# mailgun/gubernator

Measured on AMD Instinct MI355X. Metric: rate-limit decisions/sec (kernel path, inputs resident in HBM), higher is better.
Workload: dtype int64

## Files before the change

gubernator_amd/csrc/guber_front.h:

```cpp
#pragma once
#include "guber_kernels_wire.h"

constexpr uint32_t FRONT_ONE_PAIR_MAX = 49152;
struct guber_front {
    std::mutex mu;
    int device = 0;
    std::vector<guber_engine*> eng;
    std::vector<hipStream_t> streams;
    std::vector<int> stream_of;
    const guber::WireEnc* enc_hook = nullptr;
    hipStream_t rs = nullptr, rs2 = nullptr, os = nullptr, last_os = nullptr; int n_own_streams = 1; bool out_on_eval = false; uint32_t out_delay = 0, one_pair_max = FRONT_ONE_PAIR_MAX; bool rs_borrowed = false;
    uint32_t cap = 0, depth = 0, max_key = 0;
    uint32_t seq = 0;
    DevBuf<uint16_t> rt_table, rt_exs; DevBuf<uint64_t> rt_exh; RouteRule rule{}; bool have_rule = false;
    struct Slot {
        DevBuf<uint8_t> mem; CohBuf<FrontHost> host;
        FrIn in{};
        uint8_t *o_status = nullptr, *o_err = nullptr; int64_t *o_limit = nullptr, *o_remaining = nullptr, *o_reset = nullptr;
        hipEvent_t ev_in = nullptr, ev_out = nullptr, ev_a = nullptr; bool out_recorded = false;
        std::vector<std::unique_ptr<EvalHook>> hooks;
        CohBuf<uint8_t> h_margs; DevBuf<uint8_t> d_margs;
        uint32_t seq = 0, n = 0;
        int64_t gen = -1;
        bool dispatched = false;
    };
    std::vector<Slot> slots;
    uint64_t generations = 0, forced_flushes = 0, host_waits = 0; double host_wait_ms = 0;
    bool pre_routed = false;
    struct GenSpan { hipEvent_t a, b; };
    std::vector<GenSpan> gen_spans;
};

static size_t front_col(size_t bytes) { return (bytes + 63) & ~(size_t)63; }
struct FrontGen { guber_batch_t b; uint32_t key_stride = 0; const uint32_t* key_len = nullptr; };

extern "C" void guber_front_destroy(guber_front_t* f) {
    if (!f) return;
    (void)hipSetDevice(f->device);
    for (hipStream_t st : {f->rs, f->rs2, f->os}) if (st) (void)hipStreamSynchronize(st);
    for (auto st : f->streams) (void)hipStreamSynchronize(st);
    for (auto& s : f->slots) {
        s.mem.release(); s.host.release(); s.h_margs.release(); s.d_margs.release();
        if (s.ev_in) (void)hipEventDestroy(s.ev_in);
        if (s.ev_out) (void)hipEventDestroy(s.ev_out);
        for (auto& h : s.hooks) if (h && h->ev) (void)hipEventDestroy(h->ev);
    }
    f->rt_table.release(); f->rt_exs.release(); f->rt_exh.release();
    if (f->rs2 && f->rs2 != f->rs) (void)hipStreamDestroy(f->rs2);
    if (f->os && f->os != f->rs) (void)hipStreamDestroy(f->os);
    if (f->rs && !f->rs_borrowed) (void)hipStreamDestroy(f->rs);
    delete f;
}

static int front_set_rule(guber_front* f, const guber_route_rule_t* rule) {
    if (rule->n_shards == 0 || rule->per == 0 || !rule->table || rule->n_shards > 4096 || (rule->ex_cells & (rule->ex_cells - 1)) ||
        (rule->ex_n && (!rule->ex_hash || !rule->ex_shard || rule->ex_n >= rule->ex_cells)))
        return fail(GUBER_E_INVALID_ARG, "malformed route rule");
    const size_t slots = (size_t)rule->n_shards * rule->per, cells = rule->ex_cells ? rule->ex_cells : 1;
    if (f->rt_table.ensure(slots) || f->rt_exh.ensure(cells) || f->rt_exs.ensure(cells)) return GUBER_E_NOMEM;
    hipError_t he = hipStreamSynchronize(f->rs);
    if (he == hipSuccess && f->rs2) he = hipStreamSynchronize(f->rs2);
    if (he == hipSuccess) he = hipMemcpy(f->rt_table.p, rule->table, slots * 2, hipMemcpyHostToDevice);
    if (he == hipSuccess && rule->ex_n) he = hipMemcpy(f->rt_exh.p, rule->ex_hash, cells * 8, hipMemcpyHostToDevice);
    if (he == hipSuccess && rule->ex_n) he = hipMemcpy(f->rt_exs.p, rule->ex_shard, cells * 2, hipMemcpyHostToDevice);
    if (he != hipSuccess) { f->have_rule = false; return fail(GUBER_E_HIP, "guber_front: rule upload", he); }
    f->rule = RouteRule{rule->n_shards, rule->per, rule->ex_cells, rule->ex_n, rule->global_engine, rule->step, rule->inv_step, rule->inv_sub,
                        f->rt_table.p, (const unsigned long long*)f->rt_exh.p, f->rt_exs.p};
    f->have_rule = true;
    return 0;
}

extern "C" int guber_front_create(guber_engine_t* const* engines, uint32_t n_engines, const guber_route_rule_t* rule, uint32_t max_n,
                                  uint32_t depth, guber_front_t** out) {
    if (!engines || !out || !n_engines || n_engines > (uint32_t)MULTI_MEM_MAX) return fail(GUBER_E_INVALID_ARG, "1 .. 16 engines per front");
    if (n_engines > 1 && !rule) return fail(GUBER_E_INVALID_ARG, "a front over several engines needs the placement's rule");
    if (max_n == 0 || max_n > FR_MAX_N) return fail(GUBER_E_BATCH_TOO_LARGE, "a generation holds at most 4 194 304 requests");
    if (depth == 0) depth = 4;
    if (depth < 3 || depth > 16) return fail(GUBER_E_INVALID_ARG, "3 .. 16 generations in flight");
    std::unique_ptr<guber_front, void (*)(guber_front*)> f(new guber_front(), [](guber_front* p) { guber_front_destroy(p); });
    for (uint32_t j = 0; j < n_engines; ++j) {
        guber_engine* e = engines[j];
        if (!e) return fail(GUBER_E_INVALID_ARG, "null engine");
        if (e->device != engines[0]->device) return fail(GUBER_E_INVALID_ARG, "the engines of a front live on one device");
        for (uint32_t q = 0; q < j; ++q) if (engines[q] == e) return fail(GUBER_E_INVALID_ARG, "an engine twice in one front");
        f->eng.push_back(e);
        int si = -1;
        for (size_t q = 0; q < f->streams.size(); ++q) if (f->streams[q] == e->stream) si = (int)q;
        if (si < 0) { si = (int)f->streams.size(); f->streams.push_back(e->stream); }
        f->stream_of.push_back(si);
        f->max_key = j == 0 ? e->max_key : std::min(f->max_key, e->max_key);
    }
    f->device = engines[0]->device; f->cap = max_n; f->depth = depth;
    if (hipSetDevice(f->device) != hipSuccess) return fail(GUBER_E_HIP, "hipSetDevice");
    HIPCHK(hipStreamCreateWithFlags(&f->rs, hipStreamNonBlocking));
    f->n_own_streams = 1;
    if (const char* v = guber_lab_env("GUBER_FRONT_STREAMS")) f->n_own_streams = std::max(1, std::min(3, atoi(v)));
    f->out_on_eval = true;
    if (const char* v = guber_lab_env("GUBER_FRONT_OUT_ON_EVAL")) f->out_on_eval = atoi(v) != 0;
    if (const char* v = guber_lab_env("GUBER_FRONT_OUT_DELAY")) f->out_delay = (uint32_t)std::max(0, std::min(2, atoi(v)));
    if (const char* v = guber_lab_env("GUBER_FRONT_ONE_PAIR_MAX")) f->one_pair_max = (uint32_t)strtoul(v, nullptr, 10);
    f->rs2 = f->os = f->rs;
    if (f->n_own_streams >= 2) HIPCHK(hipStreamCreateWithFlags(&f->os, hipStreamNonBlocking));
    if (f->n_own_streams >= 3) HIPCHK(hipStreamCreateWithFlags(&f->rs2, hipStreamNonBlocking));
    if (rule) { const int rc = front_set_rule(f.get(), rule); if (rc) return rc; }
    else f->rule = RouteRule{1, 1, 0, 0, -1, 0, 0, 0, nullptr, nullptr, nullptr};
    const size_t cap = max_n, tiles = (cap + FR_TILE - 1) / FR_TILE;
    f->slots.resize(depth);
    for (auto& s : f->slots) {
        const size_t bytes = 3 * front_col(cap * 4 + 4) + 5 * front_col(cap * 8) + front_col(cap * 4) + 2 * front_col(cap) +
                             3 * front_col(cap * 8) + 2 * front_col(cap) +
                             front_col(cap * FR_KEY_COPY_MAX + 64) +
                             front_col(cap * 2) + 2 * front_col(tiles * MULTI_MEM_MAX * 4) + front_col(sizeof(FrontCtl));
        if (s.mem.ensure(bytes) || s.host.ensure(1)) return GUBER_E_NOMEM;
        if (f->streams.size() == 1 && n_engines > 1 && (s.h_margs.ensure(sizeof(MultiArgsMem)) || s.d_margs.ensure(sizeof(MultiArgsMem)))) return GUBER_E_NOMEM;
        uint8_t* p = s.mem.p;
        FrIn& A = s.in;
        A.d_key_off = (uint32_t*)p; p += front_col(cap * 4 + 4); A.d_key_len = (uint32_t*)p; p += front_col(cap * 4 + 4); A.d_fwd = (uint32_t*)p; p += front_col(cap * 4 + 4);
        A.d_hits = (int64_t*)p; p += front_col(cap * 8); A.d_limit = (int64_t*)p; p += front_col(cap * 8); A.d_duration = (int64_t*)p; p += front_col(cap * 8);
        A.d_burst = (int64_t*)p; p += front_col(cap * 8); A.d_created_at = (int64_t*)p; p += front_col(cap * 8);
        A.d_behavior = (uint32_t*)p; p += front_col(cap * 4); A.d_algorithm = p; p += front_col(cap); A.d_is_owner = p; p += front_col(cap);
        s.o_limit = (int64_t*)p; p += front_col(cap * 8); s.o_remaining = (int64_t*)p; p += front_col(cap * 8); s.o_reset = (int64_t*)p; p += front_col(cap * 8);
        s.o_status = p; p += front_col(cap); s.o_err = p; p += front_col(cap);
        A.d_keys = p; p += front_col(cap * FR_KEY_COPY_MAX + 64);
        A.er = (uint16_t*)p; p += front_col(cap * 2);
        A.tile_cnt = (uint32_t*)p; p += front_col(tiles * MULTI_MEM_MAX * 4); A.tile_base = (uint32_t*)p; p += front_col(tiles * MULTI_MEM_MAX * 4);
        A.ctl = (FrontCtl*)p; p += front_col(sizeof(FrontCtl));
        A.host = s.host.p;
        memset((void*)s.host.p, 0, sizeof(FrontHost));
        HIPCHK(hipMemsetAsync(A.ctl, 0, sizeof(FrontCtl), f->rs));
        HIPCHK(hipMemsetAsync(A.d_keys, 0, front_col(cap * FR_KEY_COPY_MAX + 64), f->rs));
        HIPCHK(hipEventCreateWithFlags(&s.ev_in, hipEventDisableTiming));
        HIPCHK(hipEventCreateWithFlags(&s.ev_out, hipEventDisableTiming));
        for (size_t q = 0; q < f->streams.size(); ++q) {
            s.hooks.emplace_back(new EvalHook());
            HIPCHK(hipEventCreateWithFlags(&s.hooks.back()->ev, hipEventDisableTiming));
            s.hooks.back()->st = f->streams[q];
        }
    }
    HIPCHK(hipStreamSynchronize(f->rs));
    *out = f.release();
    return GUBER_OK;
}

static int front_route_on(guber_front* f, hipStream_t st) {
    std::lock_guard<std::mutex> lk(f->mu);
    if (f->generations || f->pre_routed || f->n_own_streams != 1) return fail(GUBER_E_INVALID_ARG, "guber_front: the routing stream is chosen before the first generation");
    if (hipSetDevice(f->device) != hipSuccess) return fail(GUBER_E_HIP, "hipSetDevice");
    HIPCHK(hipStreamSynchronize(f->rs));
    HIPCHK(hipStreamDestroy(f->rs));
    f->rs = f->rs2 = f->os = st; f->rs_borrowed = true;
    return 0;
}

extern "C" int guber_front_set_rule(guber_front_t* f, const guber_route_rule_t* rule) {
    if (!f || !rule) return fail(GUBER_E_INVALID_ARG, "null argument");
    std::lock_guard<std::mutex> lk(f->mu);
    if (hipSetDevice(f->device) != hipSuccess) return fail(GUBER_E_HIP, "hipSetDevice");
    return front_set_rule(f, rule);
}

static int front_route(guber_front* f, guber_front::Slot& s, const FrontGen* fg, int64_t gen) {
    const guber_batch_t* b = &fg->b;
    hipStream_t rs = (gen & 1) ? f->rs2 : f->rs;
    if (s.out_recorded) { HIPCHK(hipStreamWaitEvent(rs, s.ev_out, 0)); s.out_recorded = false; }
    s.gen = gen; s.n = b->n; s.dispatched = false;
    s.seq = ++f->seq ? f->seq : ++f->seq;
    for (auto& h : s.hooks) { h->outstanding.store(1); h->recorded.store(false); }
    if (b->n == 0) return 0;
    FrIn& A = s.in;
    A.n = b->n; A.n_engines = (uint32_t)f->eng.size(); A.max_key = f->max_key; A.seq = s.seq;
    A.key_bytes = b->key_bytes; A.key_off = b->key_off; A.key_stride = fg->key_stride; A.key_len = fg->key_len; A.hits = b->hits; A.limit = b->limit; A.duration = b->duration;
    A.burst = b->burst; A.created_at = b->created_at; A.behavior = b->behavior; A.algorithm = b->algorithm; A.is_owner = b->is_owner;
    A.R = f->rule;
    const uint32_t tiles = (b->n + FR_TILE - 1u) / FR_TILE;
    guber_engine* e0 = f->eng[0];
    std::unique_lock<std::mutex> pl(e0->mu, std::defer_lock);
    if (e0->profiling) pl.lock();
    s.ev_a = nullptr;
    if (e0->profiling) { s.ev_a = e0->get_event(); (void)hipEventRecord(s.ev_a, rs); }
    e0->span_begin(KT_FR_COUNT, b->n, rs);
    hipLaunchKernelGGL(k_fr_count, dim3(tiles), dim3(FR_TILE), 0, rs, A);
    e0->span_end();
    e0->span_begin(KT_FR_SCAN, b->n, rs);
    hipLaunchKernelGGL(k_fr_scan, dim3(MULTI_MEM_MAX / 4), dim3(FR_SCAN_T), 0, rs, A, tiles, (tiles + FR_SCAN_T - 1) / FR_SCAN_T);
    e0->span_end();
    e0->span_begin(KT_FR_SCATTER, b->n, rs);
    hipLaunchKernelGGL(k_fr_scatter, dim3(tiles), dim3(256), 0, rs, A);
    e0->span_end();
    if (hipGetLastError() != hipSuccess) return fail(GUBER_E_HIP, "kernel launch");
    HIPCHK(hipEventRecord(s.ev_in, rs));
    return 0;
}

static int front_out(guber_front* f, guber_front::Slot& s, guber_result_t* r) {
    if (s.n == 0) return 0;
    hipStream_t os = f->out_on_eval ? f->streams[(size_t)s.gen % f->streams.size()] : f->os;
    f->last_os = os;
    for (auto& h : s.hooks) if (h->st != os) HIPCHK(hipStreamWaitEvent(os, h->ev, 0));
    FrOut O{};
    O.n = s.n; O.fwd = s.in.d_fwd;
    O.d_status = s.o_status; O.d_err = s.o_err; O.d_limit = s.o_limit; O.d_remaining = s.o_remaining; O.d_reset_time = s.o_reset;
    O.status = r->status; O.err = r->err; O.limit = r->limit; O.remaining = r->remaining; O.reset_time = r->reset_time;
    guber_engine* e0 = f->eng[0];
    std::unique_lock<std::mutex> pl(e0->mu, std::defer_lock);
    if (e0->profiling) pl.lock();
    e0->span_begin(KT_FR_OUT, s.n, os);
    if (f->enc_hook) {
        guber::WireEnc E = *f->enc_hook;
        E.fwd = O.fwd; E.d_status = O.d_status; E.d_err = O.d_err; E.d_limit = O.d_limit; E.d_remaining = O.d_remaining; E.d_reset = O.d_reset_time;
        hipLaunchKernelGGL(guber::k_wire_enc, dim3(E.nrpc), dim3(guber::WE_T), 0, os, E);
    } else
    hipLaunchKernelGGL(k_fr_out, dim3((s.n + FR_TILE - 1u) / FR_TILE), dim3(256), 0, os, O);
    e0->span_end();
    if (s.ev_a) { hipEvent_t evb = e0->get_event(); (void)hipEventRecord(evb, os); f->gen_spans.push_back({s.ev_a, evb}); s.ev_a = nullptr; }
    if (hipGetLastError() != hipSuccess) return fail(GUBER_E_HIP, "kernel launch");
    if (os != f->rs) { HIPCHK(hipEventRecord(s.ev_out, os)); s.out_recorded = true; }
    return 0;
}

static bool front_evals_launched(const guber_front::Slot& s) {
    for (auto& h : s.hooks) if (!h->recorded.load(std::memory_order_acquire)) return false;
    return true;
}

static int front_eval(guber_front* f, const FrontGen* gens, guber_result_t* results, uint32_t count, uint32_t* done, hipEvent_t after = nullptr);
extern "C" int guber_front_eval_dev(guber_front_t* f, const guber_batch_t* gens, guber_result_t* results, uint32_t count, uint32_t* done) {
    if (done) *done = 0;
    if (!f || (count && (!gens || !results))) return fail(GUBER_E_INVALID_ARG, "null argument");
    std::vector<FrontGen> g(count);
    for (uint32_t k = 0; k < count; ++k) {
        const int rc = check_batch_args(&gens[k], &results[k]);
        if (rc) return rc;
        g[k].b = gens[k];
    }
    return front_eval(f, g.data(), results, count, done);
}
static int front_eval(guber_front* f, const FrontGen* gens, guber_result_t* results, uint32_t count, uint32_t* done, hipEvent_t after) {
    if (done) *done = 0;
    for (uint32_t k = 0; k < count; ++k) {
        if (gens[k].b.n > f->cap) return fail(GUBER_E_BATCH_TOO_LARGE, "generation larger than the front was created for");
        if (gens[k].b.greg_expire || gens[k].b.greg_duration) return fail(GUBER_E_INVALID_ARG, "a front takes its calendar intervals from the device");
        if (gens[k].key_stride & 7u) return fail(GUBER_E_INVALID_ARG, "key rows are a multiple of 8 bytes apart");
        clear_aggregates(results[k]);
    }
    std::lock_guard<std::mutex> lk(f->mu);
    if (hipSetDevice(f->device) != hipSuccess) return fail(GUBER_E_HIP, "hipSetDevice");
    const uint32_t ne = (uint32_t)f->eng.size(), D = f->depth, ahead = D - 2;
    PendSet pendset;
    bool any_ep = false;
    for (auto* e : f->eng) any_ep = any_ep || e->fuse_ep;
    PendSet* const ps = any_ep ? &pendset : nullptr;
    struct Dispatching { bool on; Dispatching(bool o) : on(o) { if (on) ++tl_ep_dispatcher; } ~Dispatching() { if (on) --tl_ep_dispatcher; } } dispatching(any_ep);
    uint32_t next_route = 0, next_out = 0, enq = 0;
    int rc = 0;
    uint64_t fp[4] = {0, 0, 0, 0};
    struct FpSpan { uint64_t* a; uint64_t t0; explicit FpSpan(uint64_t* x) : a(x), t0(dp_now()) {} ~FpSpan() { if (g_dprof) *a += dp_now() - t0; } };
    const uint64_t g0 = f->generations;
    auto slot_of = [&](uint32_t k) -> guber_front::Slot& { return f->slots[(g0 + k) % D]; };
    auto drain_outs = [&](uint32_t upto, bool force) -> int {
        while (next_out < upto) {
            guber_front::Slot& s = slot_of(next_out);
            if (!s.dispatched) break;
            if (s.n && !front_evals_launched(s)) {
                if (!force) break;
                f->forced_flushes++;
                const int r2 = pendset.flush_all();
                if (r2) return r2;
                if (!front_evals_launched(s)) return fail(GUBER_E_HIP, "guber_front: an evaluation was not launched");
            }
            const int r3 = front_out(f, s, &results[next_out]);
            if (r3) return r3;
            ++next_out;
            if (done) *done = next_out;
        }
        return 0;
    };
    std::vector<std::vector<GroupItem>> fifo(ne);
    std::vector<EvalHook*> hook_of(ne, nullptr);
    for (uint32_t k = 0; k < count && !rc; ++k) {
        while (next_route < count && next_route <= k + ahead && !rc) {
            if (next_route >= D) { rc = drain_outs(next_route - D + 1, true); if (rc) break; }
            if (next_route == 0 && f->pre_routed) f->pre_routed = false;
            else { FpSpan sp(&fp[0]); rc = front_route(f, slot_of(next_route), &gens[next_route], (int64_t)f->generations + next_route); }
            ++next_route;
        }
        if (rc) break;
        guber_front::Slot& s = slot_of(k);
        const guber_batch_t* b = &gens[k].b;
        if (s.n) {
            auto reported = [&]() {
                for (int q = 0; q <= MULTI_MEM_MAX; ++q)
                    if ((uint32_t)(__atomic_load_n((volatile unsigned long long*)&s.host.p->w[q], __ATOMIC_ACQUIRE) >> 32) != s.seq) return false;
                return true;
            };
            if (!reported()) {
                FpSpan sp(&fp[1]);
                const auto t0 = std::chrono::steady_clock::now();
                f->host_waits++;
                uint32_t spins = 0;
                while (!reported()) {
                    if (++spins > 2000) {
                        std::this_thread::yield();
                        if ((spins & 0x3ffu) == 0 && hipStreamQuery((s.gen & 1) ? f->rs2 : f->rs) != hipErrorNotReady && !reported()) {
                            rc = fail(GUBER_E_HIP, "guber_front: the routing of a generation did not report"); break;
                        }
                    }
                }
                f->host_wait_ms += std::chrono::duration<double, std::milli>(std::chrono::steady_clock::now() - t0).count();
                if (rc) break;
            }
            uint32_t counts[MULTI_MEM_MAX];
            for (int q = 0; q < MULTI_MEM_MAX; ++q) counts[q] = (uint32_t)s.host.p->w[q];
            const bool packed = !((uint32_t)s.host.p->w[MULTI_MEM_MAX] >> 8 & 1u);
            for (auto st : f->streams) { if (hipStreamWaitEvent(st, s.ev_in, 0) != hipSuccess) { rc = fail(GUBER_E_HIP, "hipStreamWaitEvent"); break; } }
            if (rc) break;
            uint32_t base = 0, total = 0;
            for (uint32_t j = 0; j < ne; ++j) {
                fifo[j].clear();
                hook_of[j] = s.hooks[f->stream_of[j]].get();
                const uint32_t nj = counts[j];
                total += nj;
                guber_engine* e = f->eng[j];
                const uint32_t cap_e = std::max<uint32_t>(1u, std::min<uint32_t>(e->fast_cap ? e->fast_cap : e->max_batch, e->max_batch));
                const uint32_t np = (nj + cap_e - 1) / cap_e;
                uint32_t piece = np > 1 ? ((nj + np - 1) / np + 255u) & ~255u : cap_e;
                if (piece > cap_e) piece = cap_e;
                for (uint32_t pos = 0; pos < nj; pos += piece) {
                    const uint32_t len = std::min(piece, nj - pos), d0 = base + pos;
                    const FrIn& A = s.in;
                    BatchView B{len, 0, packed ? A.d_keys : b->key_bytes, A.d_key_off + d0, A.d_hits + d0, A.d_limit + d0, A.d_duration + d0,
                                b->burst ? A.d_burst + d0 : nullptr, b->created_at ? A.d_created_at + d0 : nullptr,
                                A.d_algorithm + d0, A.d_behavior + d0, b->is_owner ? A.d_is_owner + d0 : nullptr, nullptr, nullptr, b->now_ms,
                                0, packed ? nullptr : A.d_key_len + d0};
                    fifo[j].push_back(GroupItem{B, ResultView{s.o_status + d0, s.o_limit + d0, s.o_remaining + d0, s.o_reset + d0, s.o_err + d0}});
                }
                base += nj;
            }
            if (total != s.n) { rc = fail(GUBER_E_HIP, "guber_front: the shares do not add up to the generation"); break; }
            bool one_pair = f->streams.size() == 1 && ne > 1 && s.h_margs.p && s.n <= f->one_pair_max;
            guber_engine* og[MULTI_MEM_MAX]; GroupItem oi[MULTI_MEM_MAX]; int on = 0;
            for (uint32_t j = 0; j < ne && one_pair; ++j) {
                if (fifo[j].empty()) continue;
                one_pair = fifo[j].size() == 1 && can_fuse(f->eng[j], fifo[j][0].B.n);
                og[on] = f->eng[j]; oi[on] = fifo[j][0]; ++on;
            }
            if (one_pair && on > 1) {
                FpSpan sp(&fp[2]);
                rc = pendset.flush_all();
                int r1 = rc ? rc : launch_group_mem(og, oi, on, &enq, (MultiArgsMem*)s.h_margs.p, (MultiArgsMem*)s.d_margs.p);
                if (r1 == 1) r1 = dispatch_rounds(f->eng.data(), ne, fifo, ps, &enq, hook_of.data());
                rc = r1;
            } else { FpSpan sp(&fp[2]); rc = dispatch_rounds(f->eng.data(), ne, fifo, ps, &enq, hook_of.data()); }
        }
        s.dispatched = true;
        for (auto& h : s.hooks) h->launched();
        if (rc) break;
        { FpSpan sp(&fp[3]); rc = drain_outs(k + 1 > f->out_delay ? k + 1 - f->out_delay : 0, false); }
    }
    {
        for (uint32_t k = 0; k < next_route; ++k) {
            guber_front::Slot& s = slot_of(k);
            if (k >= next_out && !s.dispatched) { s.dispatched = true; s.n = 0; for (auto& h : s.hooks) h->launched(); }
        }
        const int rcf = pendset.flush_all();
        if (!rc) rc = rcf;
        const int rco = drain_outs(next_route, true);
        if (!rc) rc = rco;
    }
    f->generations += next_out;
    if (after && !rc && hipEventRecord(after, f->last_os ? f->last_os : f->rs) != hipSuccess) rc = fail(GUBER_E_HIP, "hipEventRecord");
    if (g_dprof && next_out) {
        fprintf(stderr, "[front] %u generations; per generation: routing enqueue %.2f us, waiting for the shares' sizes %.2f, dispatch %.2f, answers %.2f\n", next_out,
                fp[0] / 1e3 / next_out, fp[1] / 1e3 / next_out, fp[2] / 1e3 / next_out, fp[3] / 1e3 / next_out);
        if (tl_dp[6]) fprintf(stderr, "[front dispatch] %llu batches in %llu groups; per batch: wait-for-progress %.2f us, locks %.2f, preludes+plans %.2f, argument blocks %.2f, launches %.2f\n",
                (unsigned long long)tl_dp[6], (unsigned long long)tl_dp[5], tl_dp[0] / 1e3 / tl_dp[6], tl_dp[1] / 1e3 / tl_dp[6], tl_dp[2] / 1e3 / tl_dp[6],
                tl_dp[3] / 1e3 / tl_dp[6], tl_dp[4] / 1e3 / tl_dp[6]);
        for (auto& v : tl_dp) v = 0;
    }
    return rc;
}

static int front_route_ahead(guber_front* f, const FrontGen* g) {
    if (g->b.n > f->cap) return fail(GUBER_E_BATCH_TOO_LARGE, "generation larger than the front was created for");
    if (g->key_stride & 7u) return fail(GUBER_E_INVALID_ARG, "key rows are a multiple of 8 bytes apart");
    std::lock_guard<std::mutex> lk(f->mu);
    if (f->pre_routed) return fail(GUBER_E_INVALID_ARG, "guber_front: a generation is routed ahead already");
    if (hipSetDevice(f->device) != hipSuccess) return fail(GUBER_E_HIP, "hipSetDevice");
    const int rc = front_route(f, f->slots[f->generations % f->depth], g, (int64_t)f->generations);
    if (!rc) f->pre_routed = true;
    return rc;
}
static bool front_routed_ahead_ready(guber_front* f) {
    std::lock_guard<std::mutex> lk(f->mu);
    if (!f->pre_routed) return true;
    guber_front::Slot& s = f->slots[f->generations % f->depth];
    if (s.n == 0) return true;
    for (int q = 0; q <= MULTI_MEM_MAX; ++q)
        if ((uint32_t)(__atomic_load_n((volatile unsigned long long*)&s.host.p->w[q], __ATOMIC_ACQUIRE) >> 32) != s.seq) return false;
    return true;
}

extern "C" int guber_front_synchronize(guber_front_t* f) {
    if (!f) return fail(GUBER_E_INVALID_ARG, "null front");
    std::lock_guard<std::mutex> lk(f->mu);
    if (hipSetDevice(f->device) != hipSuccess) return fail(GUBER_E_HIP, "hipSetDevice");
    for (auto st : f->streams) HIPCHK(hipStreamSynchronize(st));
    for (hipStream_t st : {f->rs, f->rs2, f->os}) HIPCHK(hipStreamSynchronize(st));
    return GUBER_OK;
}

extern "C" int guber_front_latencies(guber_front_t* f, float* us, uint32_t cap, uint32_t* n_out) {
    if (!f || !n_out) return fail(GUBER_E_INVALID_ARG, "null argument");
    std::lock_guard<std::mutex> lk(f->mu);
    if (hipSetDevice(f->device) != hipSuccess) return fail(GUBER_E_HIP, "hipSetDevice");
    HIPCHK(hipStreamSynchronize(f->os));
    uint32_t n = 0;
    guber_engine* e0 = f->eng[0];
    std::lock_guard<std::mutex> lk2(e0->mu);
    for (auto& g : f->gen_spans) {
        float ms = 0;
        if (hipEventElapsedTime(&ms, g.a, g.b) == hipSuccess && us && n < cap) us[n] = ms * 1e3f;
        ++n;
        e0->event_pool.push_back(g.a); e0->event_pool.push_back(g.b);
    }
    f->gen_spans.clear();
    *n_out = n;
    return GUBER_OK;
}

extern "C" void* guber_front_stream(guber_front_t* f) { return f ? (void*)f->os : nullptr; }

extern "C" int guber_front_stats(guber_front_t* f, guber_front_stats_t* out) {
    if (!f || !out) return fail(GUBER_E_INVALID_ARG, "null argument");
    std::lock_guard<std::mutex> lk(f->mu);
    out->generations = f->generations; out->forced_flushes = f->forced_flushes; out->host_waits = f->host_waits;
    out->host_wait_us = (uint64_t)(f->host_wait_ms * 1e3);
    return GUBER_OK;
}
```

gubernator_amd/csrc/guber_kernels_front.h:

```cpp
#pragma once

namespace guber {

constexpr uint32_t FR_PER = 4;
constexpr uint32_t FR_TILE = 256 * FR_PER;
constexpr uint32_t FR_RANK_BITS = 10;
static_assert((1u << FR_RANK_BITS) >= FR_TILE && (MULTI_MEM_MAX << FR_RANK_BITS) <= 65536, "engine and rank share sixteen bits");
constexpr uint32_t FR_SCAN_T = 1024;
constexpr uint32_t FR_SCAN_PER = 4;
constexpr uint32_t FR_MAX_N = FR_SCAN_T * FR_SCAN_PER * FR_TILE;
constexpr uint32_t FR_KEY_COPY_MAX = 32;

struct FrontCtl {
    uint32_t tot[MULTI_MEM_MAX];
    uint32_t ragged_seq;
    uint32_t pad_[15];
};
struct FrontHost { unsigned long long w[MULTI_MEM_MAX + 1]; unsigned long long pad_[15]; };
static_assert(sizeof(FrontHost) == 256, "four lines of pinned memory per slot");

struct FrIn {
    uint32_t n, n_engines, max_key, seq;
    const uint8_t* key_bytes; const uint32_t* key_off;
    uint32_t key_stride; const uint32_t* key_len;
    const int64_t *hits, *limit, *duration, *burst, *created_at; const uint32_t* behavior; const uint8_t *algorithm, *is_owner;
    uint16_t* er; uint32_t* tile_cnt; uint32_t* tile_base; FrontCtl* ctl; FrontHost* host;
    uint32_t *d_key_off, *d_key_len, *d_fwd; int64_t *d_hits, *d_limit, *d_duration, *d_burst, *d_created_at; uint32_t* d_behavior; uint8_t *d_algorithm, *d_is_owner;
    uint8_t* d_keys;
    RouteRule R;
};
static_assert(sizeof(FrIn) <= 4096, "kernel arguments are limited to 4 KB");
__device__ __forceinline__ uint32_t fr_key_off(const FrIn& A, uint32_t i) { return A.key_stride ? i * A.key_stride : A.key_off[i]; }
__device__ __forceinline__ uint32_t fr_key_len(const FrIn& A, uint32_t i, uint32_t off) { return A.key_stride ? A.key_len[i] : A.key_off[i + 1] - off; }
__device__ __forceinline__ uint32_t fr_len0(const FrIn& A) { return A.key_stride ? A.key_len[0] : A.key_off[1] - A.key_off[0]; }

__global__ __launch_bounds__(FR_TILE) void k_fr_count(FrIn A) {
    __shared__ uint32_t wtot[FR_TILE / 64][MULTI_MEM_MAX];
    const uint32_t tid = threadIdx.x, lane = tid & 63u, wave = tid >> 6, i = blockIdx.x * FR_TILE + tid;
    if (tid < (FR_TILE / 64) * MULTI_MEM_MAX) (&wtot[0][0])[tid] = 0u;
    uint32_t e = 0xffu;
    if (i < A.n) {
        const uint32_t len0 = fr_len0(A);
        const uint32_t o0 = A.key_stride ? 0u : A.key_off[0], oend = A.key_stride ? A.n * A.key_stride : A.key_off[A.n];
        const uint32_t off_g = A.key_stride ? i * A.key_stride : o0 + i * len0;
        uint64_t kw[4] = {0, 0, 0, 0};
        const bool spec = len0 != 0 && len0 < 32 && (A.key_stride ? A.key_stride >= 32u : (uint64_t)off_g + 32 <= (uint64_t)oend + 8);
        if (spec) { const uint8_t* kp = A.key_bytes + off_g; kw[0] = ld_key_word(kp); kw[1] = ld_key_word(kp + 8); kw[2] = ld_key_word(kp + 16); kw[3] = ld_key_word(kp + 24); }
        const uint32_t off = fr_key_off(A, i), len = fr_key_len(A, i, off);
        e = 0;
        if (A.R.global_engine >= 0 && A.behavior && (A.behavior[i] & 2u)) e = (uint32_t)A.R.global_engine;
        else if (len != 0 && len <= A.max_key && A.R.n_shards > 1)
            e = route_engine(A.R, (spec && off == off_g && len == len0) ? xxhash64_words4(kw, len, 0) : xxhash64(A.key_bytes + off, len, 0));
        if (e >= A.n_engines) e = 0;
        if (len != len0 || off != off_g || len0 == 0 || len0 > FR_KEY_COPY_MAX) {
            if (__hip_atomic_load(&A.ctl->ragged_seq, __ATOMIC_RELAXED, __HIP_MEMORY_SCOPE_AGENT) != A.seq) atomicExch(&A.ctl->ragged_seq, A.seq);
        }
    }
    __syncthreads();
    unsigned long long same = __ballot(e <= 15u);
#pragma unroll
    for (uint32_t b = 0; b < 4; ++b) { const unsigned long long m = __ballot((e >> b) & 1u); same &= ((e >> b) & 1u) ? m : ~m; }
    if (e > 15u) same = 0ull;
    uint32_t rank = (uint32_t)__popcll(same & ((1ull << lane) - 1ull));
    if (same && rank == 0) wtot[wave][e] = (uint32_t)__popcll(same);
    __syncthreads();
    if (i < A.n) {
        for (uint32_t w = 0; w < wave; ++w) rank += wtot[w][e];
        A.er[i] = (uint16_t)(e << FR_RANK_BITS | rank);
    }
    if (tid < MULTI_MEM_MAX) {
        uint32_t c = 0;
        for (uint32_t w = 0; w < FR_TILE / 64; ++w) c += wtot[w][tid];
        A.tile_cnt[blockIdx.x * MULTI_MEM_MAX + tid] = c;
    }
}

__global__ __launch_bounds__(FR_SCAN_T) void k_fr_scan(FrIn A, uint32_t nt, uint32_t per) {
    __shared__ uint32_t wsum[FR_SCAN_T / 64][4];
    const uint32_t tid = threadIdx.x, lane = tid & 63u, wave = tid >> 6, q = blockIdx.x;
    const uint32_t t0 = tid * per, t1 = t0 + per < nt ? t0 + per : nt;
    uint32_t m0 = 0, m1 = 0, m2 = 0, m3 = 0;
#pragma unroll 1
    for (uint32_t t = t0; t < t1; ++t) { const uint4 v = ((const uint4*)(A.tile_cnt + (size_t)t * MULTI_MEM_MAX))[q]; m0 += v.x; m1 += v.y; m2 += v.z; m3 += v.w; }
    const uint32_t i0 = (uint32_t)wave_incl_scan_i32((int)m0), i1 = (uint32_t)wave_incl_scan_i32((int)m1);
    const uint32_t i2 = (uint32_t)wave_incl_scan_i32((int)m2), i3 = (uint32_t)wave_incl_scan_i32((int)m3);
    if (lane == 63) { wsum[wave][0] = i0; wsum[wave][1] = i1; wsum[wave][2] = i2; wsum[wave][3] = i3; }
    __syncthreads();
    uint32_t e0 = i0 - m0, e1 = i1 - m1, e2 = i2 - m2, e3 = i3 - m3;
    for (uint32_t w = 0; w < wave; ++w) { e0 += wsum[w][0]; e1 += wsum[w][1]; e2 += wsum[w][2]; e3 += wsum[w][3]; }
#pragma unroll 1
    for (uint32_t t = t0; t < t1; ++t) {
        const uint4 v = ((const uint4*)(A.tile_cnt + (size_t)t * MULTI_MEM_MAX))[q];
        ((uint4*)(A.tile_base + (size_t)t * MULTI_MEM_MAX))[q] = make_uint4(e0, e1, e2, e3);
        e0 += v.x; e1 += v.y; e2 += v.z; e3 += v.w;
    }
    if (tid < 4) {
        uint32_t all = 0;
        for (uint32_t w = 0; w < FR_SCAN_T / 64; ++w) all += wsum[w][tid];
        A.ctl->tot[4 * q + tid] = all;
        __hip_atomic_store(&A.host->w[4 * q + tid], (unsigned long long)A.seq << 32 | all, __ATOMIC_RELAXED, __HIP_MEMORY_SCOPE_SYSTEM);
    }
    if (q == 0 && tid == 0) {
        const uint32_t ragged = __hip_atomic_load(&A.ctl->ragged_seq, __ATOMIC_RELAXED, __HIP_MEMORY_SCOPE_AGENT) == A.seq ? 1u : 0u;
        const uint32_t len0 = fr_len0(A);
        __hip_atomic_store(&A.host->w[MULTI_MEM_MAX], (unsigned long long)A.seq << 32 | ragged << 8 | (len0 < 255u ? len0 : 255u), __ATOMIC_RELAXED, __HIP_MEMORY_SCOPE_SYSTEM);
    }
}

__global__ __launch_bounds__(256) void k_fr_scatter(FrIn A) {
    __shared__ uint32_t sbase[MULTI_MEM_MAX];
    if (threadIdx.x < MULTI_MEM_MAX) {
        uint32_t b = 0;
        for (uint32_t k = 0; k < threadIdx.x; ++k) b += A.ctl->tot[k];
        sbase[threadIdx.x] = b;
    }
    __syncthreads();
    const uint32_t tile = blockIdx.x, i0 = tile * FR_TILE + threadIdx.x;
    const bool packed = A.ctl->ragged_seq != A.seq;
    uint32_t er[FR_PER], o0[FR_PER], o1[FR_PER], beh[FR_PER]; int64_t hits[FR_PER], limit[FR_PER], duration[FR_PER]; uint8_t algo[FR_PER];
#pragma unroll
    for (int k = 0; k < FR_PER; ++k) {
        const uint32_t i = i0 + k * 256u;
        if (i >= A.n) { er[k] = 0xffffffffu; continue; }
        er[k] = A.er[i]; o0[k] = fr_key_off(A, i); o1[k] = o0[k] + fr_key_len(A, i, o0[k]);
        hits[k] = A.hits[i]; limit[k] = A.limit[i]; duration[k] = A.duration[i];
        beh[k] = A.behavior ? A.behavior[i] : 0u; algo[k] = A.algorithm ? A.algorithm[i] : (uint8_t)0;
    }
#pragma unroll
    for (int k = 0; k < FR_PER; ++k) {
        const uint32_t i = i0 + k * 256u;
        if (er[k] == 0xffffffffu) continue;
        const uint32_t e = er[k] >> FR_RANK_BITS, rank = er[k] & ((1u << FR_RANK_BITS) - 1u);
        const uint32_t d = sbase[e] + A.tile_base[tile * MULTI_MEM_MAX + e] + rank;
        A.d_fwd[i] = d < A.n ? d : 0u;
        if (d >= A.n) continue;
        A.d_hits[d] = hits[k]; A.d_limit[d] = limit[k]; A.d_duration[d] = duration[k]; A.d_behavior[d] = beh[k]; A.d_algorithm[d] = algo[k];
        if (A.burst) A.d_burst[d] = A.burst[i];
        if (A.created_at) A.d_created_at[d] = A.created_at[i];
        if (A.is_owner) A.d_is_owner[d] = A.is_owner[i];
        if (packed) {
            const uint32_t len = o1[k] - o0[k];
            const uint8_t* src = A.key_bytes + o0[k]; uint8_t* dst = A.d_keys + (size_t)d * len;
            if (len >= 8) {
                uint32_t b = 0;
                for (; b + 8 <= len; b += 8) { const uint64_t w = ld_key_word(src + b); __builtin_memcpy(dst + b, &w, 8); }
                if (b < len) { const uint64_t w = ld_key_word(src + len - 8); __builtin_memcpy(dst + len - 8, &w, 8); }
            } else {
                const uint64_t w = ld_key_word(src);
                for (uint32_t q = 0; q < len; ++q) dst[q] = (uint8_t)(w >> (8 * q));
            }
            A.d_key_off[d] = d * len;
            if (d == A.n - 1) A.d_key_off[A.n] = A.n * len;
        } else {
            A.d_key_off[d] = o0[k]; A.d_key_len[d] = o1[k] - o0[k];
        }
    }
}

struct FrOut {
    uint32_t n; const uint32_t* fwd;
    const uint8_t *d_status, *d_err; const int64_t *d_limit, *d_remaining, *d_reset_time;
    uint8_t *status, *err; int64_t *limit, *remaining, *reset_time;
};
__global__ __launch_bounds__(256) void k_fr_out(FrOut A) {
    const uint32_t i0 = blockIdx.x * FR_TILE + threadIdx.x;
    uint32_t d[FR_PER]; uint8_t st[FR_PER], er[FR_PER]; int64_t l[FR_PER], r[FR_PER], t[FR_PER];
#pragma unroll
    for (int k = 0; k < FR_PER; ++k) d[k] = i0 + k * 256u < A.n ? A.fwd[i0 + k * 256u] : 0xffffffffu;
#pragma unroll
    for (int k = 0; k < FR_PER; ++k) {
        if (d[k] == 0xffffffffu) continue;
        st[k] = A.d_status[d[k]]; er[k] = A.d_err[d[k]]; l[k] = A.d_limit[d[k]]; r[k] = A.d_remaining[d[k]]; t[k] = A.d_reset_time[d[k]];
    }
#pragma unroll
    for (int k = 0; k < FR_PER; ++k) {
        if (d[k] == 0xffffffffu) continue;
        const uint32_t i = i0 + k * 256u;
        A.limit[i] = l[k]; A.remaining[i] = r[k]; A.reset_time[i] = t[k]; A.status[i] = st[k]; A.err[i] = er[k];
    }
}

}
```

Measured before the change: 4.838 billion.

## Stage front scatter and gather through shared memory for coalesced column writes

The scatter and output kernels now compute per-tile engine bases in shared memory and permute each column through a double-buffered LDS staging array. Global reads and writes then land on contiguous sorted destinations instead of random per-element scatter/gather addresses. The output kernel rebuilds the permutation from the engine/rank codes instead of reading the forward index array. This adds barriers and LDS traffic per column, and relies on each tile's destinations being contiguous per engine. Packed keys are assumed to share one fixed length.

```diff
diff --git a/gubernator_amd/csrc/guber_front.h b/gubernator_amd/csrc/guber_front.h
--- a/gubernator_amd/csrc/guber_front.h
+++ b/gubernator_amd/csrc/guber_front.h
@@ -198,7 +198,7 @@
     f->last_os = os;
     for (auto& h : s.hooks) if (h->st != os) HIPCHK(hipStreamWaitEvent(os, h->ev, 0));
     FrOut O{};
-    O.n = s.n; O.fwd = s.in.d_fwd;
+    O.n = s.n; O.er = s.in.er; O.tile_cnt = s.in.tile_cnt; O.tile_base = s.in.tile_base; O.ctl = s.in.ctl;
     O.d_status = s.o_status; O.d_err = s.o_err; O.d_limit = s.o_limit; O.d_remaining = s.o_remaining; O.d_reset_time = s.o_reset;
     O.status = r->status; O.err = r->err; O.limit = r->limit; O.remaining = r->remaining; O.reset_time = r->reset_time;
     guber_engine* e0 = f->eng[0];
@@ -207,7 +207,7 @@
     e0->span_begin(KT_FR_OUT, s.n, os);
     if (f->enc_hook) {
         guber::WireEnc E = *f->enc_hook;
-        E.fwd = O.fwd; E.d_status = O.d_status; E.d_err = O.d_err; E.d_limit = O.d_limit; E.d_remaining = O.d_remaining; E.d_reset = O.d_reset_time;
+        E.fwd = s.in.d_fwd; E.d_status = O.d_status; E.d_err = O.d_err; E.d_limit = O.d_limit; E.d_remaining = O.d_remaining; E.d_reset = O.d_reset_time;
         hipLaunchKernelGGL(guber::k_wire_enc, dim3(E.nrpc), dim3(guber::WE_T), 0, os, E);
     } else
     hipLaunchKernelGGL(k_fr_out, dim3((s.n + FR_TILE - 1u) / FR_TILE), dim3(256), 0, os, O);
diff --git a/gubernator_amd/csrc/guber_kernels_front.h b/gubernator_amd/csrc/guber_kernels_front.h
--- a/gubernator_amd/csrc/guber_kernels_front.h
+++ b/gubernator_amd/csrc/guber_kernels_front.h
@@ -107,77 +107,168 @@
     }
 }
 
+struct FrTile { uint32_t lbase[MULTI_MEM_MAX + 1], dofs[MULTI_MEM_MAX]; };
+__device__ __forceinline__ void fr_tile_bases(FrTile& T, const FrontCtl* ctl, const uint32_t* tile_cnt, const uint32_t* tile_base, uint32_t tile) {
+    const uint32_t e = threadIdx.x;
+    if (e < MULTI_MEM_MAX) {
+        const uint32_t* cnt = tile_cnt + (size_t)tile * MULTI_MEM_MAX;
+        uint32_t s = 0, l = 0;
+        for (uint32_t k = 0; k < e; ++k) { s += ctl->tot[k]; l += cnt[k]; }
+        T.lbase[e] = l; T.dofs[e] = s + tile_base[(size_t)tile * MULTI_MEM_MAX + e] - l;
+        if (e == MULTI_MEM_MAX - 1) T.lbase[MULTI_MEM_MAX] = l + cnt[e];
+    }
+    __syncthreads();
+}
+__device__ __forceinline__ uint32_t fr_engine_of(const FrTile& T, uint32_t j) {
+    uint32_t e = 0;
+#pragma unroll
+    for (uint32_t q = 1; q < MULTI_MEM_MAX; ++q) e += T.lbase[q] <= j ? 1u : 0u;
+    return e;
+}
+__device__ __forceinline__ void fr_sorted_places(const FrTile& T, uint32_t n, uint32_t (&dd)[FR_PER]) {
+    const uint32_t cnt = T.lbase[MULTI_MEM_MAX] < FR_TILE ? T.lbase[MULTI_MEM_MAX] : FR_TILE;
+#pragma unroll
+    for (int k = 0; k < FR_PER; ++k) {
+        const uint32_t j = threadIdx.x + k * 256u, d = T.dofs[fr_engine_of(T, j)] + j;
+        dd[k] = j < cnt && d < n ? d : 0xffffffffu;
+    }
+}
+
 __global__ __launch_bounds__(256) void k_fr_scatter(FrIn A) {
-    __shared__ uint32_t sbase[MULTI_MEM_MAX];
-    if (threadIdx.x < MULTI_MEM_MAX) {
-        uint32_t b = 0;
-        for (uint32_t k = 0; k < threadIdx.x; ++k) b += A.ctl->tot[k];
-        sbase[threadIdx.x] = b;
-    }
-    __syncthreads();
-    const uint32_t tile = blockIdx.x, i0 = tile * FR_TILE + threadIdx.x;
+    __shared__ FrTile T;
+    __shared__ uint64_t stg[2][FR_TILE];
+    const uint32_t tile = blockIdx.x, tid = threadIdx.x, i0 = tile * FR_TILE + tid;
+    fr_tile_bases(T, A.ctl, A.tile_cnt, A.tile_base, tile);
     const bool packed = A.ctl->ragged_seq != A.seq;
-    uint32_t er[FR_PER], o0[FR_PER], o1[FR_PER], beh[FR_PER]; int64_t hits[FR_PER], limit[FR_PER], duration[FR_PER]; uint8_t algo[FR_PER];
+    const uint32_t len0 = fr_len0(A), ko0 = A.key_stride ? 0u : A.key_off[0], kstep = A.key_stride ? A.key_stride : len0;
+    uint32_t p[FR_PER], o0[FR_PER], klen[FR_PER]; uint64_t hits[FR_PER], limit[FR_PER], duration[FR_PER], misc[FR_PER], kw[FR_PER];
+    auto word_at = [](uint32_t w, uint32_t len) { return 8u * w + 8u <= len || len < 8u ? 8u * w : len - 8u; };
 #pragma unroll
     for (int k = 0; k < FR_PER; ++k) {
         const uint32_t i = i0 + k * 256u;
-        if (i >= A.n) { er[k] = 0xffffffffu; continue; }
-        er[k] = A.er[i]; o0[k] = fr_key_off(A, i); o1[k] = o0[k] + fr_key_len(A, i, o0[k]);
-        hits[k] = A.hits[i]; limit[k] = A.limit[i]; duration[k] = A.duration[i];
-        beh[k] = A.behavior ? A.behavior[i] : 0u; algo[k] = A.algorithm ? A.algorithm[i] : (uint8_t)0;
-    }
-#pragma unroll
-    for (int k = 0; k < FR_PER; ++k) {
-        const uint32_t i = i0 + k * 256u;
-        if (er[k] == 0xffffffffu) continue;
-        const uint32_t e = er[k] >> FR_RANK_BITS, rank = er[k] & ((1u << FR_RANK_BITS) - 1u);
-        const uint32_t d = sbase[e] + A.tile_base[tile * MULTI_MEM_MAX + e] + rank;
+        p[k] = 0xffffffffu; o0[k] = klen[k] = 0; hits[k] = limit[k] = duration[k] = misc[k] = kw[k] = 0;
+        if (i >= A.n) continue;
+        const uint32_t er = A.er[i];
+        if (packed) { o0[k] = ko0 + i * kstep; klen[k] = len0; kw[k] = ld_key_word(A.key_bytes + o0[k]); }
+        else { o0[k] = fr_key_off(A, i); klen[k] = fr_key_len(A, i, o0[k]); }
+        hits[k] = (uint64_t)A.hits[i]; limit[k] = (uint64_t)A.limit[i]; duration[k] = (uint64_t)A.duration[i];
+        misc[k] = (A.behavior ? A.behavior[i] : 0u) | (uint64_t)(A.algorithm ? A.algorithm[i] : (uint8_t)0) << 32 | (uint64_t)(A.is_owner ? A.is_owner[i] : (uint8_t)0) << 40;
+        const uint32_t e = er >> FR_RANK_BITS;
+        p[k] = T.lbase[e] + (er & ((1u << FR_RANK_BITS) - 1u));
+        const uint32_t d = T.dofs[e] + p[k];
         A.d_fwd[i] = d < A.n ? d : 0u;
-        if (d >= A.n) continue;
-        A.d_hits[d] = hits[k]; A.d_limit[d] = limit[k]; A.d_duration[d] = duration[k]; A.d_behavior[d] = beh[k]; A.d_algorithm[d] = algo[k];
-        if (A.burst) A.d_burst[d] = A.burst[i];
-        if (A.created_at) A.d_created_at[d] = A.created_at[i];
-        if (A.is_owner) A.d_is_owner[d] = A.is_owner[i];
-        if (packed) {
-            const uint32_t len = o1[k] - o0[k];
-            const uint8_t* src = A.key_bytes + o0[k]; uint8_t* dst = A.d_keys + (size_t)d * len;
-            if (len >= 8) {
-                uint32_t b = 0;
-                for (; b + 8 <= len; b += 8) { const uint64_t w = ld_key_word(src + b); __builtin_memcpy(dst + b, &w, 8); }
-                if (b < len) { const uint64_t w = ld_key_word(src + len - 8); __builtin_memcpy(dst + len - 8, &w, 8); }
-            } else {
-                const uint64_t w = ld_key_word(src);
-                for (uint32_t q = 0; q < len; ++q) dst[q] = (uint8_t)(w >> (8 * q));
+    }
+    uint32_t dd[FR_PER];
+    fr_sorted_places(T, A.n, dd);
+    uint32_t turn = 0;
+    auto through = [&](const uint64_t (&v)[FR_PER], uint64_t (&o)[FR_PER]) {
+        uint64_t* buf = stg[turn++ & 1u];
+#pragma unroll
+        for (int k = 0; k < FR_PER; ++k) if (p[k] < FR_TILE) buf[p[k]] = v[k];
+        __syncthreads();
+#pragma unroll
+        for (int k = 0; k < FR_PER; ++k) o[k] = dd[k] != 0xffffffffu ? buf[threadIdx.x + k * 256u] : 0ull;
+    };
+    auto column = [&](const uint64_t (&v)[FR_PER], int64_t* dst) {
+        uint64_t o[FR_PER];
+        through(v, o);
+#pragma unroll
+        for (int k = 0; k < FR_PER; ++k) if (dd[k] != 0xffffffffu) dst[dd[k]] = (int64_t)o[k];
+    };
+    uint64_t opt[FR_PER] = {0, 0, 0, 0}, o[FR_PER];
+    auto request = [&](const int64_t* src) {
+#pragma unroll
+        for (int k = 0; k < FR_PER; ++k) if (p[k] != 0xffffffffu) opt[k] = (uint64_t)src[i0 + k * 256u];
+    };
+    column(hits, A.d_hits);
+    column(limit, A.d_limit);
+    if (A.burst) request(A.burst);
+    column(duration, A.d_duration);
+    if (A.burst) column(opt, A.d_burst);
+    if (A.created_at) request(A.created_at);
+    through(misc, o);
+#pragma unroll
+    for (int k = 0; k < FR_PER; ++k) {
+        if (dd[k] == 0xffffffffu) continue;
+        A.d_behavior[dd[k]] = (uint32_t)o[k]; A.d_algorithm[dd[k]] = (uint8_t)(o[k] >> 32);
+        if (A.is_owner) A.d_is_owner[dd[k]] = (uint8_t)(o[k] >> 40);
+    }
+    if (A.created_at) column(opt, A.d_created_at);
+    if (packed) {
+        const uint32_t nw = (len0 + 7u) >> 3;
+        for (uint32_t w = 0; w < nw; ++w) {
+            uint64_t next[FR_PER] = {0, 0, 0, 0};
+            if (w + 1 < nw) {
+#pragma unroll
+                for (int k = 0; k < FR_PER; ++k) if (p[k] != 0xffffffffu) next[k] = ld_key_word(A.key_bytes + o0[k] + word_at(w + 1, len0));
             }
-            A.d_key_off[d] = d * len;
-            if (d == A.n - 1) A.d_key_off[A.n] = A.n * len;
-        } else {
-            A.d_key_off[d] = o0[k]; A.d_key_len[d] = o1[k] - o0[k];
+            through(kw, o);
+#pragma unroll
+            for (int k = 0; k < FR_PER; ++k) {
+                kw[k] = next[k];
+                if (dd[k] == 0xffffffffu) continue;
+                uint8_t* dst = A.d_keys + (size_t)dd[k] * len0;
+                if (len0 >= 8) __builtin_memcpy(dst + word_at(w, len0), &o[k], 8);
+                else for (uint32_t q = 0; q < len0; ++q) dst[q] = (uint8_t)(o[k] >> (8 * q));
+            }
         }
+#pragma unroll
+        for (int k = 0; k < FR_PER; ++k) {
+            if (dd[k] == 0xffffffffu) continue;
+            A.d_key_off[dd[k]] = dd[k] * len0;
+            if (dd[k] == A.n - 1) A.d_key_off[A.n] = A.n * len0;
+        }
+    } else {
+        uint64_t ol[FR_PER];
+#pragma unroll
+        for (int k = 0; k < FR_PER; ++k) ol[k] = o0[k] | (uint64_t)klen[k] << 32;
+        through(ol, o);
+#pragma unroll
+        for (int k = 0; k < FR_PER; ++k) if (dd[k] != 0xffffffffu) { A.d_key_off[dd[k]] = (uint32_t)o[k]; A.d_key_len[dd[k]] = (uint32_t)(o[k] >> 32); }
     }
 }
 
 struct FrOut {
-    uint32_t n; const uint32_t* fwd;
+    uint32_t n; const uint16_t* er; const uint32_t *tile_cnt, *tile_base; const FrontCtl* ctl;
     const uint8_t *d_status, *d_err; const int64_t *d_limit, *d_remaining, *d_reset_time;
     uint8_t *status, *err; int64_t *limit, *remaining, *reset_time;
 };
 __global__ __launch_bounds__(256) void k_fr_out(FrOut A) {
-    const uint32_t i0 = blockIdx.x * FR_TILE + threadIdx.x;
-    uint32_t d[FR_PER]; uint8_t st[FR_PER], er[FR_PER]; int64_t l[FR_PER], r[FR_PER], t[FR_PER];
-#pragma unroll
-    for (int k = 0; k < FR_PER; ++k) d[k] = i0 + k * 256u < A.n ? A.fwd[i0 + k * 256u] : 0xffffffffu;
-#pragma unroll
-    for (int k = 0; k < FR_PER; ++k) {
-        if (d[k] == 0xffffffffu) continue;
-        st[k] = A.d_status[d[k]]; er[k] = A.d_err[d[k]]; l[k] = A.d_limit[d[k]]; r[k] = A.d_remaining[d[k]]; t[k] = A.d_reset_time[d[k]];
-    }
-#pragma unroll
-    for (int k = 0; k < FR_PER; ++k) {
-        if (d[k] == 0xffffffffu) continue;
-        const uint32_t i = i0 + k * 256u;
-        A.limit[i] = l[k]; A.remaining[i] = r[k]; A.reset_time[i] = t[k]; A.status[i] = st[k]; A.err[i] = er[k];
-    }
-}
-
-}
+    __shared__ FrTile T;
+    __shared__ uint64_t stg[2][FR_TILE];
+    __shared__ uint16_t sse[FR_TILE];
+    const uint32_t tile = blockIdx.x, tid = threadIdx.x, i0 = tile * FR_TILE + tid;
+    fr_tile_bases(T, A.ctl, A.tile_cnt, A.tile_base, tile);
+    uint32_t dd[FR_PER], p[FR_PER]; uint16_t se[FR_PER]; int64_t l[FR_PER], r[FR_PER], t[FR_PER];
+    fr_sorted_places(T, A.n, dd);
+#pragma unroll
+    for (int k = 0; k < FR_PER; ++k) {
+        p[k] = 0xffffffffu;
+        if (i0 + k * 256u < A.n) { const uint32_t er = A.er[i0 + k * 256u]; p[k] = T.lbase[er >> FR_RANK_BITS] + (er & ((1u << FR_RANK_BITS) - 1u)); }
+        if (p[k] >= FR_TILE) p[k] = 0xffffffffu;
+        se[k] = 0; l[k] = r[k] = t[k] = 0;
+        if (dd[k] == 0xffffffffu) continue;
+        se[k] = (uint16_t)(A.d_status[dd[k]] | A.d_err[dd[k]] << 8); l[k] = A.d_limit[dd[k]]; r[k] = A.d_remaining[dd[k]]; t[k] = A.d_reset_time[dd[k]];
+    }
+#pragma unroll
+    for (int k = 0; k < FR_PER; ++k) { stg[0][tid + k * 256u] = (uint64_t)l[k]; sse[tid + k * 256u] = se[k]; }
+    __syncthreads();
+#pragma unroll
+    for (int k = 0; k < FR_PER; ++k) {
+        if (p[k] == 0xffffffffu) continue;
+        const uint32_t i = i0 + k * 256u; const uint16_t v = sse[p[k]];
+        A.limit[i] = (int64_t)stg[0][p[k]]; A.status[i] = (uint8_t)v; A.err[i] = (uint8_t)(v >> 8);
+    }
+#pragma unroll
+    for (int k = 0; k < FR_PER; ++k) stg[1][tid + k * 256u] = (uint64_t)r[k];
+    __syncthreads();
+#pragma unroll
+    for (int k = 0; k < FR_PER; ++k) if (p[k] != 0xffffffffu) A.remaining[i0 + k * 256u] = (int64_t)stg[1][p[k]];
+#pragma unroll
+    for (int k = 0; k < FR_PER; ++k) stg[0][tid + k * 256u] = (uint64_t)t[k];
+    __syncthreads();
+#pragma unroll
+    for (int k = 0; k < FR_PER; ++k) if (p[k] != 0xffffffffu) A.reset_time[i0 + k * 256u] = (int64_t)stg[0][p[k]];
+}
+
+}
```

Result: faster. 5.090 billion (median of 6 runs) (+5.2%).
